# erthward/geonomics

Hardware: AMD Instinct MI355X
Metric: individual-timesteps/sec (higher is better)
Workload: dtype u64

## Files before the change

geonomics_amd/csrc/gnx_kernels_demog.hip:

```cpp
#include "gnx_internal.h"
#include <chrono>
#include "gnx_rng.h"
#include "gnx_compact.h"
#include "gnx_half.h"
#include "gnx_xo.h"

#define BIN_BLOCKS 512

__global__ void __launch_bounds__(256)
k_bins(int64_t n, const int32_t* n_dev, const float* x, const float* y, const uint8_t* ghost,
       double inv_hww, int nbx, int nby, int32_t* partials, GnxSetWords sw) {
  extern __shared__ int32_t lds_hist[];
  if (sw.dst && blockIdx.x == 0 && threadIdx.x < 4) sw.dst[threadIdx.x] = sw.v[threadIdx.x];
  if (n_dev) n = *n_dev;
  const int nb = nbx * nby;
  for (int k = threadIdx.x; k < nb; k += blockDim.x) lds_hist[k] = 0;
  __syncthreads();
  const int64_t stride = (int64_t)gridDim.x * blockDim.x;
  for (int64_t i = (int64_t)blockIdx.x * blockDim.x + threadIdx.x; i < n; i += stride) {
    if (ghost && ghost[i]) continue;
    int hx = min(nbx - 1, (int)floor((double)x[i] * inv_hww));
    int hy = min(nby - 1, (int)floor((double)y[i] * inv_hww));
    atomicAdd(&lds_hist[hy * nbx + hx], 1);
  }
// ... 645 lines not shown
                     n_max, (const int32_t*)h->cnt_dev, (const float*)h->mid_x,
                     (const float*)h->mid_y, (const uint8_t*)nullptr, 1.0 / L.hww, L.nbx, L.nby,
                     h->fb[2], GnxSetWords{});
  hipLaunchKernelGGL(k_lattice, dim3(1), dim3(256), lds_bytes, h->stream3, L.Jx, L.Jy, L.nbx,
                     (const int32_t*)h->fb[2], L.areas, L.hww, L.cprime, h->spl_P.c,
                     (int32_t*)nullptr, 0, (unsigned long long*)nullptr, 1, 1);
  HIPCHK(hipEventRecord(h->ev_latP, h->stream3));
  HIPCHK(hipGetLastError());
  h->latP_inflight = true;
  h->fb_zero[2] = true;
  h->spl_P.valid = true;
  return 0;
}

int gnx_l_bins_adults_async(gnx_state* h, const float* d_x, const float* d_y, int64_t N) {
  if (!(h->have_sp && gnx_fused_bins(h))) {
    h->fb_adults = false;
    return 0;
  }
  const GnxLattice& L = h->lat;
  const int nb = L.nbx * L.nby;
  const int cur = h->fb_cur;
  if (!h->fb_zero[cur])
    HIPCHK(hipMemsetAsync(h->fb[cur], 0, (size_t)nb * sizeof(int32_t), h->stream));
  h->fbp_x = d_x;
  h->fbp_y = d_y;
  h->fbp_N = N;
  h->fb_pending = true;
  h->fb_zero[cur] = false;
  h->fb_adults = true;
  h->fb_count = N;
  return 0;
}

int gnx_bins_adults_launch(gnx_state* h) {
  if (!h->fb_pending) return 0;
  h->fb_pending = false;
  const GnxLattice& L = h->lat;
  const int nb = L.nbx * L.nby;
  const int64_t N = h->fbp_N;
  const int blocks = (int)std::min<int64_t>(BIN_BLOCKS, std::max<int64_t>(1, (N + 255) / 256));
  hipLaunchKernelGGL(k_bins, dim3(blocks), dim3(256), (size_t)nb * sizeof(int32_t), h->stream3, N,
                     (const int32_t*)nullptr, h->fbp_x, h->fbp_y, (const uint8_t*)nullptr,
                     1.0 / L.hww, L.nbx, L.nby, h->fb[h->fb_cur], GnxSetWords{});
  HIPCHK(hipEventRecord(h->ev_binsN, h->stream3));
  HIPCHK(hipGetLastError());
  h->binsN_inflight = true;
  return 0;
}

void gnx_bins_adults_drop(gnx_state* h) {
  if (h->fb_pending) {
    h->fb_pending = false;
    h->fb_adults = false;
  }
}

int gnx_l_density_N(gnx_state* h) {
  GnxSoA s = h->soa[h->cur];
  if (!(gnx_fused_bins(h) && h->fb_adults && h->fb_count == h->N)) {
    h->fb_adults = false;
    h->nmax_ready = false;
    h->last_N_fused = false;
    return gnx_l_density(h, h->N, s.x, s.y, &h->spl_N, nullptr);
  }
  const GnxLattice& L = h->lat;
  const int64_t nn = (int64_t)L.Jx * L.Jy;
  const size_t lat_doubles = (size_t)4 * nn + std::max(L.Jx, L.Jy) + 1;
  const int nmax_R = gnx_nmax_rows_fit(L.Jx, lat_doubles);
  const size_t lds_bytes = (lat_doubles + gnx_nmax_lds_doubles(L.Jx, nmax_R)) * sizeof(double);
  const int cur = h->fb_cur;
  if (h->fb_pending) {
    HIPCHK(hipEventRecord(h->ev_perm, h->stream));
    HIPCHK(hipStreamWaitEvent(h->stream3, h->ev_perm, 0));
    GNXCHK(gnx_bins_adults_launch(h));
  }
  if (h->binsN_inflight) {
    HIPCHK(hipStreamWaitEvent(h->stream, h->ev_binsN, 0));
    h->binsN_inflight = false;
  }
  gnx_time_begin(h);
  hipLaunchKernelGGL(k_lattice_nmax, dim3(std::max(1, std::min(h->cfg.H, GNX_LATN_BLOCKS))), dim3(256),
                     lds_bytes, h->stream, L.Jx, L.Jy, L.nbx, (const int32_t*)h->fb[cur], L.areas,
                     L.hww, L.cprime, h->spl_N.c, h->cfg.W, h->cfg.H, h->nmax2 + cur,
                     h->fb[cur ^ 1], h->nmax2 + (cur ^ 1), (int32_t*)nullptr, (double*)nullptr,
                     GnxPubWords{}, nmax_R, gnx_nmax_scan_min());
  gnx_time_end(h, GNX_K_DENSITY, (double)h->N * 8.0);
  HIPCHK(hipGetLastError());
  h->spl_N.valid = true;
  h->nmax_cur = h->nmax2 + cur;
  h->nmax_ready = true;
  h->fb_zero[cur] = false;
  h->fb_zero[cur ^ 1] = true;
  h->fb_cur = cur ^ 1;
  h->fb_adults = false;
  h->last_N_fused = true;
  return 0;
}

bool gnx_l_lattices_tiled(gnx_state* h, bool have_pairs, const GnxPubWords& pub) {
  const GnxLattice& L = h->lat;
  const int64_t nn = (int64_t)L.Jx * L.Jy;
  const size_t lat_doubles = (size_t)4 * nn + std::max(L.Jx, L.Jy) + 1;
  const int nmax_R = gnx_nmax_rows_fit(L.Jx, lat_doubles);
  const size_t lds_bytes = (lat_doubles + gnx_nmax_lds_doubles(L.Jx, nmax_R)) * sizeof(double);
  if (lds_bytes > 64 * 1024 || !h->nmax_bits || !h->nmax_zeroed) return false;
  gnx_time_begin(h);
  hipLaunchKernelGGL(k_lattice_nmax,
                     dim3(std::max(1, std::min(h->cfg.H, GNX_LATN_BLOCKS)) + (have_pairs ? 1 : 0)),
                     dim3(256), lds_bytes, h->stream, L.Jx, L.Jy, L.nbx,
                     (const int32_t*)h->bin_partials, L.areas, L.hww, L.cprime, h->spl_N.c, h->cfg.W,
                     h->cfg.H, h->nmax_bits, (int32_t*)nullptr, (unsigned long long*)nullptr,
                     have_pairs ? h->bins_P : (int32_t*)nullptr, h->spl_P.c, pub, nmax_R, gnx_nmax_scan_min());
  gnx_time_end(h, GNX_K_DENSITY, (double)h->N * 8.0);
  h->spl_N.valid = true;
  h->spl_P.valid = have_pairs;
  h->nmax_cur = h->nmax_bits;
  h->nmax_ready = true;
  h->nmax_zeroed = false;
  return true;
}

int gnx_l_death_probs(gnx_state* h, bool with_selection) {
  int64_t N = h->N;
  if (N == 0) return 0;
  SplineC SN = make_splinec(h, h->spl_N), SP = make_splinec(h, h->spl_P);
  GNXCHK(gnx_wait_latP(h));
  gnx_time_begin(h);
  if (!h->nmax_ready) GNXCHK(launch_nmax(h));
  h->nmax_ready = false;
  hipLaunchKernelGGL(k_death_probs, dim3(gnx_grid(N, 256)), dim3(256), 0, h->stream,
                     make_deathp(h, with_selection), make_demp(h), SN, SP, h->soa[h->cur], h->rast,
                     gnx_trait_tab(h), h->delet_s, h->nmax_cur, h->p_death, h->d_cell);
  gnx_time_end(h, GNX_K_DEATH, (double)N * (28.0 + 8.0 * h->cfg.n_traits));
  HIPCHK(hipGetLastError());
  return 0;
}

__global__ void __launch_bounds__(256)
k_alive(int64_t N, const double* p_death, const uint8_t* dead_in, const int64_t* id,
        const uint8_t* ghost, const int32_t* grow, long long step, unsigned long long seed,
        int32_t* alive, int32_t* dead_row, int32_t* cnt, int stride, int64_t xo_first,
        int32_t* zero_jobs, const GnxDD* __restrict__ dd, GnxScanOut scan) {
  __shared__ int lds[16];
  __shared__ int lds2[8];
  const int64_t base = (int64_t)blockIdx.x * GNX_CB;
  if (dd) {
    N = (int64_t)dd->N + dd->B;
    step = dd->step;
    if (xo_first >= 0) xo_first = dd->N;
  }
  if (zero_jobs && blockIdx.x == 0 && threadIdx.x == 0) *zero_jobs = 0;
  bool fa[4], fd[4], fx[4];
#pragma unroll
  for (int r = 0; r < 4; ++r) {
    const int64_t i = base + r * 256 + threadIdx.x;
    fa[r] = fd[r] = fx[r] = false;
    if (i < N) {
      bool dead;
      const bool g = ghost[i] != 0;
      if (g) {
        dead = true;
      } else if (dead_in) {
        dead = dead_in[i] != 0;
      } else {
        uint4 rr = gnx_rand4(seed, (unsigned long long)id[i], step, OP_DEATH, 0);
        dead = (double)gnx_u01(rr.x) < p_death[i];
      }
      fa[r] = !dead;
      fd[r] = dead && !g && grow[i] >= 0;
      fx[r] = !dead && xo_first >= 0 && i >= xo_first && grow[i] < 0;
      alive[i] = (fa[r] ? 1 : 0) | (fx[r] ? 2 : 0);
      dead_row[i] = fd[r] ? 1 : 0;
    }
  }
  int rank[4], ta, td, tx;
  gnx_block_ranks(fa, rank, ta, lds);
  gnx_block_ranks(fd, rank, td, lds);
  gnx_block_ranks(fx, rank, tx, lds);
  if (scan.ticket) {
    const int v[3] = {ta, td, tx};
    gnx_count_and_scan<3>(v, cnt, scan, lds2);
    return;
  }
  if (threadIdx.x == 0) {
    cnt[blockIdx.x] = ta;
    cnt[stride + blockIdx.x] = td;
    cnt[2 * stride + blockIdx.x] = tx;
  }
}

struct GnxXoPlan {
  int32_t row;
  int32_t pop, job;
  int32_t prow[2];
  int32_t mixsel[2];
  int32_t ks[2];
  int32_t pad;
};

__global__ void __launch_bounds__(256)
k_xo_jobs_surv(int64_t N, int64_t first, int32_t* __restrict__ grow,
               const int32_t* __restrict__ alive, const int32_t* __restrict__ blk_off3,
               const int32_t* __restrict__ off_parent, const int32_t* __restrict__ off_keys,
               const uint8_t* __restrict__ off_start, const int32_t* __restrict__ free_rows,
               int64_t n_free, GnxHalves H, const int32_t* __restrict__ bp_off,
               const int32_t* __restrict__ bp_loci, int32_t* __restrict__ n_jobs,
               GnxXoPlan* __restrict__ plan) {
  __shared__ int lds[16];
  __shared__ int s_pop, s_job;
  const int64_t b = first / GNX_CB + blockIdx.x;
  const int64_t base = b * GNX_CB;
  bool fx[4];
#pragma unroll
  for (int r = 0; r < 4; ++r) {
    const int64_t i = base + r * 256 + threadIdx.x;
    fx[r] = i < N && (alive[i] & 2) != 0;
  }
  int rank[4], tot;
  gnx_block_ranks(fx, rank, tot, lds);
  const int32_t boff = blk_off3[b];
  const int NB = H.NB;
  const unsigned int all = (1u << NB) - 1u;
  int32_t row[4], prow[4][2], ks[4][2];
  int32_t par[4][2], key[4][2], st[4][2];
#pragma unroll
  for (int r = 0; r < 4; ++r) {
    const int64_t i = base + r * 256 + threadIdx.x;
    const int64_t k = fx[r] ? i - first : 0;
    row[r] = free_rows[n_free - 1 - (fx[r] ? boff + rank[r] : 0)];
#pragma unroll
    for (int p = 0; p < 2; ++p) {
      par[r][p] = off_parent[2 * k + p];
      key[r][p] = off_keys[2 * k + p];
      st[r][p] = off_start[2 * k + p];
    }
  }
  int32_t b0[4][2], b1[4][2];
#pragma unroll
  for (int r = 0; r < 4; ++r) {
    const int64_t i = base + r * 256 + threadIdx.x;
    if (fx[r]) grow[i] = row[r];
    else row[r] = -1;
#pragma unroll
    for (int p = 0; p < 2; ++p) {
      prow[r][p] = grow[par[r][p]];
      b0[r][p] = bp_off ? bp_off[key[r][p]] : 0;
      b1[r][p] = bp_off ? bp_off[key[r][p] + 1] : 0;
    }
  }
  unsigned int mixed[4][2], sel[4][2];
  int cf[4], cj[4];
#pragma unroll
  for (int r = 0; r < 4; ++r) {
    cf[r] = cj[r] = 0;
#pragma unroll
    for (int p = 0; p < 2; ++p) {
      if (!fx[r]) prow[r][p] = -1;
      ks[r][p] = key[r][p] * 2 + st[r][p];
      mixed[r][p] = all;
      sel[r][p] = 0u;
      if (fx[r] && prow[r][p] >= 0 && bp_off)
        gnx_block_masks(bp_loci + b0[r][p], b1[r][p] - b0[r][p], st[r][p], NB, H.BW, mixed[r][p],
                        sel[r][p]);
      if (fx[r]) {
        const int nf = __popc(mixed[r][p] & all);
        cf[r] += nf;
        cj[r] += prow[r][p] >= 0 ? nf : 0;
      }
    }
  }
  int of[4], oj[4], tf, tj;
  gnx_block_sums(cf, of, tf, lds);
  gnx_block_sums(cj, oj, tj, lds);
  if (threadIdx.x == 0) {
    s_pop = tf ? atomicSub(H.top, tf) : 0;
    s_job = tj ? atomicAdd(n_jobs, tj) : 0;
  }
  __syncthreads();
  const int pop0 = s_pop, job0 = s_job;
#pragma unroll
  for (int r = 0; r < 4; ++r) {
    const int64_t i = base + r * 256 + threadIdx.x;
    if (i < first || i >= N) continue;
    GnxXoPlan P;
    P.row = fx[r] ? row[r] : -1;
    P.pop = pop0 - 1 - of[r];
    P.job = job0 + oj[r];
#pragma unroll
    for (int p = 0; p < 2; ++p) {
      P.prow[p] = prow[r][p];
      P.mixsel[p] = (mixed[r][p] & 0xffffu) | (sel[r][p] << 16);
      P.ks[p] = ks[r][p];
    }
    plan[i - first] = P;
  }
}

__global__ void __launch_bounds__(256)
k_xo_jobs_write(int64_t B, GnxHalves H, const GnxXoPlan* __restrict__ plan,
                GnxXoJob* __restrict__ jobs) {
  const int NB = H.NB;
  const int64_t t = (int64_t)blockIdx.x * blockDim.x + threadIdx.x;
  if (t >= B * 2 * NB) return;
  const int64_t k = t / (2 * NB);
  const int rem = (int)(t - k * 2 * NB);
  const int p = rem / NB, q = rem - p * NB;
  const GnxXoPlan P = plan[k];
  if (P.row < 0) return;
  const unsigned int all = (1u << NB) - 1u;
  const unsigned int m0 = P.mixsel[0] & all, m1 = P.mixsel[1] & all;
  const unsigned int mixed = p ? m1 : m0, sel = (unsigned int)P.mixsel[p] >> 16;
  const unsigned int below = (1u << q) - 1u;
  const bool local = P.prow[p] >= 0;
  const int64_t lb = ((int64_t)P.row * 2 + p) * NB + q;
  const int64_t ph0 = (int64_t)(local ? P.prow[p] : 0) * 2 * NB;
  if ((mixed >> q) & 1u) {
    const int fr = (p ? __popc(m0) : 0) + __popc(mixed & below);
    const int jr = (p && P.prow[0] >= 0 ? __popc(m0) : 0) + __popc(mixed & below);
    const int32_t dst = H.stack[P.pop - fr];
    H.hmap[lb] = (int32_t)((uint32_t)dst | GNX_OWN);
    if (local) {
      GnxXoJob j;
      j.ph0 = GNX_BLK(H.hmap[ph0 + q]);
// ... 467 lines not shown
                       lds, lds2);
  }
}

__global__ void __launch_bounds__(256)
k_fill(int64_t cap, const int32_t* __restrict__ n_move, const int32_t* __restrict__ holes,
       const int32_t* __restrict__ movers, const int32_t* __restrict__ cnts, GnxSoA a, int n_layers,
       int n_traits, int tbw, const int32_t* __restrict__ rows_tmp, int32_t* __restrict__ free_rows,
       int64_t n_free, int has_rows, int xo, int32_t* __restrict__ newslot,
       const GnxDD* __restrict__ dd) {
  if (dd) n_free = dd->n_free;
  const int64_t stride = (int64_t)gridDim.x * blockDim.x;
  const int64_t t0 = (int64_t)blockIdx.x * blockDim.x + threadIdx.x;
  const int64_t H = *n_move;
  for (int64_t r = t0; r < H; r += stride) {
    const int64_t i = movers[r], k = holes[r];
    GnxRec rec = gnx_rec_load(a, i, cap, n_layers, n_traits, tbw);
    rec.ghost = 0;
    if (newslot) newslot[i] = (int32_t)k;
    gnx_rec_store(a, k, cap, n_layers, n_traits, tbw, rec);
    gnx_rec_rest(a, i, a, k, cap, n_layers, n_traits, tbw);
  }
  if (has_rows) {
    if (xo) n_free -= cnts[2];
    const int64_t D = cnts[1];
    for (int64_t r = t0; r < D; r += stride) free_rows[n_free + r] = rows_tmp[r];
  }
}

static bool jobs_fused_ok(const gnx_state* h) { return h->NB <= GNX_JF_NB; }

void gnx_launch_xo_jobs_surv(gnx_state* h, int64_t first_slot, const int32_t* d_alive,
                             const int32_t* d_blk_off, int buf) {
  const int64_t N = h->N;
  const int nbj = (int)((N - 1) / GNX_CB - first_slot / GNX_CB + 1);
  if (jobs_fused_ok(h)) {
    launch_jobs_fused(h, first_slot, d_alive, d_blk_off, buf);
    return;
  }
  h->jobs_inline[buf] = false;
  hipLaunchKernelGGL(k_xo_jobs_surv, dim3(nbj), dim3(256), 0, h->stream, N, first_slot,
                     h->soa[h->cur].grow, d_alive, d_blk_off + 2 * h->blk_stride, h->off_parent,
                     h->off_keys, h->off_start, h->free_rows, h->n_free, gnx_halves(h),
                     gnx_alias_bp(h), gnx_alias_loci(h), h->n_jobs_dev[buf], (GnxXoPlan*)h->xo_plan);
  const int64_t B = N - first_slot;
  hipLaunchKernelGGL(k_xo_jobs_write, dim3(gnx_grid(B * 2 * h->NB, 256)), dim3(256), 0, h->stream,
                     B, gnx_halves(h), (const GnxXoPlan*)h->xo_plan, (GnxXoJob*)h->jobs[buf]);
}

struct GnxDDEnd {
  GnxDD* dd;
  const int32_t* cnts;
  const int32_t* half_top;
  GnxDDRec* ring;
  int has_rows, xo;
  unsigned int* ticket;
};
__device__ __forceinline__ void gnx_dd_end_step(const GnxDDEnd& E) {
  GnxDD* dd = E.dd;
  const int32_t S = E.cnts[0], freed = E.cnts[1], X = E.xo ? E.cnts[2] : 0;
  GnxDDRec r;
  r.N0 = dd->N;
  r.P = dd->P;
  r.B = dd->B;
  r.S = S;
  r.xo = X;
  const int32_t n_free = dd->n_free - X + (E.has_rows ? freed : 0);
  r.n_free = n_free;
  r.half_top = E.half_top ? *E.half_top : 0;
  r.err = dd->err;
  r.max_id = dd->max_id + dd->B;
  r.step = dd->step;
  const int32_t seq = dd->seq + 1;
  dd->N = S;
  dd->ord_n = S;
  dd->n_free = n_free;
  dd->max_id = r.max_id;
  dd->step = dd->step + 1;
  dd->seq = seq;
  dd->P = 0;
  dd->B = 0;
  GnxDDRec* slot = E.ring + ((seq - 1) % GNX_DD_RING);
  __hip_atomic_store(&slot->seq, (int64_t)0, __ATOMIC_RELAXED, __HIP_MEMORY_SCOPE_SYSTEM);
  int64_t* w = (int64_t*)slot;
  const int64_t* v = (const int64_t*)&r;
  for (int k = 1; k < (int)(sizeof(GnxDDRec) / 8); ++k)
    __hip_atomic_store(&w[k], v[k], __ATOMIC_RELAXED, __HIP_MEMORY_SCOPE_SYSTEM);
  __hip_atomic_store(&slot->seq, (int64_t)seq, __ATOMIC_RELEASE, __HIP_MEMORY_SCOPE_SYSTEM);
}

__global__ void __launch_bounds__(256)
k_ord_flags(int64_t N, int64_t ord_n, const int32_t* __restrict__ ord,
            const int32_t* __restrict__ newslot, int32_t* __restrict__ cnt, GnxScanOut S,
            const GnxDD* __restrict__ dd, const int32_t* __restrict__ alive) {
  __shared__ int lds[16];
  __shared__ int lds2[8];
  if (dd) {
    N = (int64_t)dd->N + dd->B;
    ord_n = dd->ord_n;
  }
  gnx_ord_flags_body(N, ord_n, GnxOrdF{ord, alive ? nullptr : newslot, alive, cnt, S, ord_n, 0},
                     lds, lds2);
}

__global__ void __launch_bounds__(256)
k_ord_write(int64_t N, int64_t ord_n, const int32_t* __restrict__ ord,
            const int32_t* __restrict__ newslot, const int32_t* __restrict__ off,
            int32_t* __restrict__ ord_new, const GnxDD* __restrict__ dd, GnxDDEnd E,
            int tail_explicit, const int32_t* __restrict__ alive) {
  __shared__ int lds[16];
  __shared__ int last_s;
  if (dd) {
    N = (int64_t)dd->N + dd->B;
    ord_n = tail_explicit ? N : (int64_t)dd->ord_n;
  }
  const int64_t base = (int64_t)blockIdx.x * GNX_CB;
  bool f[4];
  int32_t ns[4];
#pragma unroll
  for (int r = 0; r < 4; ++r) {
    const int64_t k = base + r * 256 + threadIdx.x;
    if (alive) {
      const int32_t slot = k < N ? (int32_t)(k < ord_n ? ord[k] : k) : -1;
      ns[r] = (slot >= 0 && (alive[slot] & 1) != 0) ? slot : -1;
    } else {
      ns[r] = k < N ? newslot[k < ord_n ? ord[k] : k] : -1;
    }
    f[r] = ns[r] >= 0;
  }
  int rank[4], tot;
  gnx_block_ranks(f, rank, tot, lds);
  const int32_t o = off[blockIdx.x];
#pragma unroll
  for (int r = 0; r < 4; ++r)
    if (f[r]) ord_new[o + rank[r]] = ns[r];
  if (!E.dd) return;
  __syncthreads();
  if (threadIdx.x == 0) {
    const unsigned int t = __hip_atomic_fetch_add(E.ticket, 1u, __ATOMIC_RELAXED, __HIP_MEMORY_SCOPE_AGENT);
    last_s = t == gridDim.x - 1u;
    if (last_s) __hip_atomic_store(E.ticket, 0u, __ATOMIC_RELAXED, __HIP_MEMORY_SCOPE_AGENT);
  }
  __syncthreads();
  if (last_s && threadIdx.x == 0) gnx_dd_end_step(E);
}

__global__ void __launch_bounds__(256)
k_dead_rows(int64_t N, const int32_t* __restrict__ dead_row, const int32_t* __restrict__ blk_off_d,
            int32_t* __restrict__ grow, const int32_t* __restrict__ cnts, int xo,
            int32_t* __restrict__ free_rows, int64_t n_free) {
  __shared__ int lds[16];
  const int64_t base = (int64_t)blockIdx.x * GNX_CB;
  bool fd[4];
#pragma unroll
  for (int r = 0; r < 4; ++r) {
    const int64_t i = base + r * 256 + threadIdx.x;
    fd[r] = i < N && dead_row[i] != 0;
  }
  int rd[4], td;
  gnx_block_ranks(fd, rd, td, lds);
  if (xo) n_free -= cnts[2];
  const int32_t od = blk_off_d[blockIdx.x];
#pragma unroll
  for (int r = 0; r < 4; ++r) {
    const int64_t i = base + r * 256 + threadIdx.x;
    if (fd[r]) {
      free_rows[n_free + od + rd[r]] = grow[i];
      grow[i] = -1;
    }
  }
}

int gnx_l_mortality(gnx_state* h, const uint8_t* d_dead_inject, int64_t* deaths_out) {
  *deaths_out = 0;
  GNXCHK(gnx_l_mortality_enqueue(h, d_dead_inject));
  return gnx_l_mortality_finish(h, deaths_out);
}

int gnx_l_mortality_enqueue(gnx_state* h, const uint8_t* d_dead_inject) {
  int64_t N = h->N;
  h->mort_wait = false;
  gnx_bins_adults_drop(h);
  if (N == 0) return 0;
  const gnx_config& c = h->cfg;
  GnxSoA a = h->soa[h->cur], b = h->soa[h->cur ^ 1];
  const int nb = (int)((N + GNX_CB - 1) / GNX_CB);
  const bool xo = h->xo_deferred;
  const int64_t xo_first = h->xo_first, xo_B = xo ? h->xo_B : 0;
  const bool ord_keep = h->ord_mode && h->ord_valid && !h->tiled;
  int32_t* zero_jobs = nullptr;
  if (xo) {
    GNXCHK(gnx_xo_prepare_jobs(h, &zero_jobs));
    GNXCHK(gnx_half_reserve(h, 2 * (int64_t)h->NB * xo_B));
  }
  gnx_time_begin(h);
  hipLaunchKernelGGL(k_alive, dim3(nb), dim3(256), 0, h->stream, N, h->p_death, d_dead_inject,
                     a.id, a.ghost, a.grow, h->step, c.seed, h->flag, h->flag2, h->blk_cnt,
                     h->blk_stride, xo ? xo_first : (int64_t)-1, zero_jobs, (const GnxDD*)nullptr,
                     GnxScanOut{});
  const bool fill = h->compact_fill && h->stream3 != nullptr && d_dead_inject == nullptr;
  const bool side_scan = fill && xo && xo_B > 0 && jobs_fused_ok(h);
  const bool lazy_common = fill && h->sp.move && h->sp.mating_radius >= 0;
  const bool lazy_tile = lazy_common && gnx_env_int("GNX_TILE_LAZY", 0) != 0 && h->tile_lazy_ok &&
                         h->tile2_mode && h->tile_R * h->tile_C > 1 && !ord_keep;
  const bool lazy = lazy_tile || (lazy_common && h->eager_move && ord_keep && h->key_bits <= 24 &&
                                  h->n_ghost == 0 && !h->tile2_mode);
  const bool move_ahead = lazy && ord_keep && h->move_ahead_ok && h->stream2 != nullptr &&
                          h->xo_launch_late;
  const bool lazy_ord = lazy && ord_keep;
  if (side_scan || lazy_ord) HIPCHK(hipEventRecord(h->ev_alive, h->stream));
  if (side_scan) {
    HIPCHK(hipStreamWaitEvent(h->stream3, h->ev_alive, 0));
    GNXCHK(gnx_block_scan(h, 3, N, h->blk_cnt, h->blk_off, h->cnt_dev, h->h_pin_dev, 0, h->stream3));
    gnx_time_end(h, GNX_K_COMPACT, 0.0);
    HIPCHK(hipEventRecord(h->ev_counts, h->stream3));
  } else {
    GNXCHK(gnx_block_scan(h, 3, N, h->blk_cnt, h->blk_off, h->cnt_dev, h->h_pin_dev));
    gnx_time_end(h, GNX_K_COMPACT, 0.0);
    HIPCHK(hipEventRecord(h->ev_counts, h->stream));
  }
  h->jobs_self_scan = side_scan;
  int has_rows = (h->genomes_assigned && c.L > 0) ? 1 : 0;
  if (fill && !lazy) {
    if (!side_scan) HIPCHK(hipStreamWaitEvent(h->stream3, h->ev_counts, 0));
    hipLaunchKernelGGL(k_fill_lists, dim3(nb), dim3(256), 0, h->stream3, N, h->flag, h->flag2,
                       h->blk_off, h->blk_stride, h->cnt_dev, a.grow, has_rows,
                       (int32_t*)h->os_ktmp, (int32_t*)h->os_ktmp + c.cap_inds / 2,
                       (int32_t*)h->os_vtmp, ord_keep ? h->newslot : nullptr, h->fill_cnt,
                       (const GnxDD*)nullptr, GnxOrdF{});
    HIPCHK(hipEventRecord(h->ev_fill, h->stream3));
  }
  if (xo) {
    h->xo_deferred = false;
    GNXCHK(gnx_l_crossover_survivors(h, xo_first, xo_B, h->flag, h->blk_off));
    h->jobs_self_scan = false;
    if (h->xo_sort_waits && h->xo_wait_at == 2) GNXCHK(gnx_xo_wait_inflight(h));
  }
  if (move_ahead) GNXCHK(gnx_l_move_ahead(h, N));
  if (ord_keep && h->ord_inflight) HIPCHK(hipStreamWaitEvent(h->stream, h->ev_ord, 0));
  auto ord_launch = [&](hipStream_t os) {
    GnxScanOut So{h->ord_off, nullptr, nullptr, 0, nullptr, h->tickets + 2, h->blk_stride};
    hipLaunchKernelGGL(k_ord_flags, dim3(nb), dim3(256), 0, os, N, h->ord_n,
                       h->ord[h->ord_cur], h->newslot, h->ord_cnt, So, (const GnxDD*)nullptr,
                       lazy ? (const int32_t*)h->flag : (const int32_t*)nullptr);
    hipLaunchKernelGGL(k_ord_write, dim3(nb), dim3(256), 0, os, N, h->ord_n,
                       h->ord[h->ord_cur], h->newslot, h->ord_off, h->ord[h->ord_cur ^ 1],
                       (const GnxDD*)nullptr, GnxDDEnd{}, 0,
                       lazy ? (const int32_t*)h->flag : (const int32_t*)nullptr);
  };
  if (move_ahead) {
    ord_launch(h->stream);
    h->ord_inflight = false;
    h->ord_covers_xo = false;
    h->ord_cur ^= 1;
  }
  gnx_time_begin(h);
  const double rec_bytes = 34.0 + 4.0 * c.n_layers + 4.0 * c.n_traits + 16.0 * h->TW;
  if (lazy) {
    if (has_rows) {
      if (side_scan) HIPCHK(hipStreamWaitEvent(h->stream, h->ev_counts, 0));
      hipLaunchKernelGGL(k_dead_rows, dim3(nb), dim3(256), 0, h->stream, N,
                         (const int32_t*)h->flag2, (const int32_t*)(h->blk_off + h->blk_stride),
                         a.grow, (const int32_t*)h->cnt_dev, xo ? 1 : 0,
                         h->free_rows, h->n_free);
    }
    gnx_time_end(h, GNX_K_COMPACT, (double)N * 8.0);
    h->holes = true;
    h->holes_N = N;
    h->holes_flagged = N;
    ++h->pc[GNX_PC_LAZY_MORT];
  } else if (fill) {
    HIPCHK(hipStreamWaitEvent(h->stream, h->ev_fill, 0));
    const int64_t guess = std::max<int64_t>(h->fill_guess * 2, 4096);
    const int fb_ = (int)std::min<int64_t>(gnx_grid(std::min<int64_t>(guess, N), 256), 8192);
    hipLaunchKernelGGL(k_fill, dim3(fb_), dim3(256), 0, h->stream, c.cap_inds, h->fill_cnt,
                       (const int32_t*)h->os_ktmp, (const int32_t*)h->os_ktmp + c.cap_inds / 2,
                       h->cnt_dev, a, c.n_layers, c.n_traits, a.tb ? 2 * h->TW : 0,
                       (const int32_t*)h->os_vtmp, h->free_rows, h->n_free, has_rows, xo ? 1 : 0,
                       ord_keep ? h->newslot : nullptr, (const GnxDD*)nullptr);
    gnx_time_end(h, GNX_K_COMPACT, (double)N * 16.0 + (double)h->fill_guess * (16.0 + 2.0 * rec_bytes));
  } else {
    hipLaunchKernelGGL(k_compact, dim3(nb), dim3(256), 0, h->stream, N, c.cap_inds, h->flag,
                       h->flag2, h->blk_off, h->blk_stride, h->cnt_dev, a, b, c.n_layers, c.n_traits,
                       a.tb ? 2 * h->TW : 0, h->free_rows, h->n_free, has_rows, xo ? 1 : 0,
                       ord_keep ? h->newslot : nullptr);
    gnx_time_end(h, GNX_K_COMPACT, (double)N * (24.0 + 2.0 * rec_bytes));
  }
  if (move_ahead) {
  } else if (ord_keep) {
    if (!lazy_ord) {
      HIPCHK(hipEventRecord(h->ev_compact, h->stream));
      HIPCHK(hipStreamWaitEvent(h->stream3, h->ev_compact, 0));
    } else if (!side_scan) {
      HIPCHK(hipStreamWaitEvent(h->stream3, h->ev_alive, 0));
    }
    if (h->ord_inflight) h->ord_inflight = false;
    ord_launch(h->stream3);
    h->ord_covers_xo = false;
    if (h->xo_sort_waits && !h->xo_last_split && h->xo_ready_buf < 0) {
      for (int k = 0; k < 2; ++k)
        if (h->xo_inflight[k]) HIPCHK(hipStreamWaitEvent(h->stream3, h->ev_xo_done[k], 0));
      h->ord_covers_xo = true;
    }
    HIPCHK(hipEventRecord(h->ev_ord, h->stream3));
    h->ord_inflight = true;
    h->ord_cur ^= 1;
  } else {
    h->ord_valid = false;
  }
  HIPCHK(hipGetLastError());
  h->mort_wait = true;
  h->mort_xo = xo;
  h->mort_fill = fill;
  h->mort_ord_keep = ord_keep;
  h->mort_has_rows = has_rows;
  h->mort_N = N;
  return 0;
}

int gnx_l_mortality_finish(gnx_state* h, int64_t* deaths_out) {
// ... 191 lines not shown
```

geonomics_amd/csrc/gnx_kernels_pop.hip:

```cpp
#include "gnx_internal.h"
#include "gnx_rng.h"
#include "gnx_compact.h"
#include "gnx_tb.h"
#include "gnx_bins.h"

static int gnx_id_bits(const gnx_state* h) {
  int b = 1;
  while (b < 40 && (h->max_id >> b) != 0) ++b;
  return b;
}
static bool gnx_ord_sort(const gnx_state* h) {
  return h->ord_mode && h->ord_valid && !h->tiled;
}

__device__ __forceinline__ int wave_min_i(int v) {
#pragma unroll
  for (int m = 32; m >= 1; m >>= 1) v = min(v, __shfl_xor(v, m));
  return v;
}
__device__ __forceinline__ int wave_max_i(int v) {
#pragma unroll
  for (int m = 32; m >= 1; m >>= 1) v = max(v, __shfl_xor(v, m));
  return v;
}
// ... 1315 lines not shown
  if (n_dev) nb = (int)(((int64_t)*n_dev + GNX_CB - 1) / GNX_CB);
  if (dd) nb = (int)(((int64_t)dd->N + GNX_CB - 1) / GNX_CB);
  const int seg = (nb + 15) / 16;
  const int b0 = wave * seg, b1 = min(nb, b0 + seg);
  int run = 0;
  for (int b = b0; b < b1; ++b) run += blk_cnt[(int64_t)b * GNX_VTN + c];
  seg_tot[wave][c] = run;
  __syncthreads();
  int before = 0, total = 0;
  for (int w = 0; w < 16; ++w) {
    const int t = seg_tot[w][c];
    before += w < wave ? t : 0;
    total += t;
  }
  run = before;
  for (int b = b0; b < b1; ++b) {
    const int v = blk_cnt[(int64_t)b * GNX_VTN + c];
    blk_off[(int64_t)b * GNX_VTN + c] = run;
    run += v;
  }
  if (wave != 0) return;
  vt_count[c] = total;
  if (local) {
    int xs = total;
#pragma unroll
    for (int d = 1; d < 64; d <<= 1) {
      const int yv = __shfl_up(xs, d);
      if (c >= d) xs += yv;
    }
    vt_base[c] = (int64_t)(xs - total) * lam;
  }
}

struct GnxGoff {
  const int64_t* goff;
  const uint8_t* cls;
  const int32_t* rank;
  const int32_t* pblk;
  const int32_t* blk_off;
  const int64_t* vt_base;
  int64_t mul;
};

int gnx_vt_buffers(gnx_state* h) {
  if (h->vt_cls) return 0;
  const size_t cap = (size_t)h->cfg.cap_inds;
  const size_t nb = cap / GNX_CB + 2;
  HIPCHK(hipMalloc((void**)&h->vt_cls, cap));
  HIPCHK(hipMalloc((void**)&h->vt_scls, cap));
  HIPCHK(hipMalloc((void**)&h->vt_blk_nz, nb * sizeof(unsigned long long)));
  HIPCHK(hipMalloc((void**)&h->vt_rank, cap * sizeof(int32_t)));
  HIPCHK(hipMalloc((void**)&h->vt_pblk, cap * sizeof(int32_t)));
  HIPCHK(hipMalloc((void**)&h->vt_blk_cnt, nb * GNX_VTN * sizeof(int32_t)));
  HIPCHK(hipMalloc((void**)&h->vt_blk_off, nb * GNX_VTN * sizeof(int32_t)));
  HIPCHK(hipMalloc((void**)&h->vt_count, (GNX_VTN + GNX_MAX_TILES + 8) * sizeof(int32_t)));
  HIPCHK(hipMemset(h->vt_count, 0, (GNX_VTN + GNX_MAX_TILES + 8) * sizeof(int32_t)));
  HIPCHK(hipMalloc((void**)&h->vt_base, GNX_VTN * sizeof(int64_t)));
  return 0;
}

static GnxVtP gnx_vtp(const gnx_state* h) {
  const int vw = h->cfg.W / GNX_VT, vh = h->cfg.H / GNX_VT;
  return GnxVtP{vw, vh, 1.0f / (float)vw, 1.0f / (float)vh};
}

static int gnx_vt_out(gnx_state* h, GnxVtOut* out) {
  *out = GnxVtOut{nullptr, nullptr, nullptr, 0, nullptr, nullptr, nullptr, nullptr, 0, 1,
                  GnxVtP{1, 1, 1.f, 1.f}};
  h->vt_fused = false;
  if (h->id_order != 1 || !h->sp.n_births_fixed || h->sp.mating_radius < 0) return 0;
  GNXCHK(gnx_vt_buffers(h));
  *out = GnxVtOut{h->vt_scls, h->vt_blk_cnt, h->vt_blk_nz, (int)(h->cfg.cap_inds / GNX_CB + 2),
                  h->vt_count, h->vt_cls, h->vt_rank, h->vt_base,
                  h->tiled ? 0 : 1, (int64_t)h->sp.n_births_lambda, gnx_vtp(h)};
  h->vt_fused = true;
  return 0;
}

int gnx_l_pair_cls(gnx_state* h, int64_t P, bool local) {
  GNXCHK(gnx_vt_buffers(h));
  GnxSoA s = h->soa[h->cur];
  if (h->sp.n_births_fixed) {
    if (!h->vt_fused && h->N > 0 && P != 0) {
      gnx_set_error("tile-major offspring ids: the pair list was made without its classification");
      return 1;
    }
    if (local != !h->tiled) {
      gnx_set_error("tile-major offspring ids: the bases' owner does not match the tile grid");
      return 1;
    }
    h->vt_mul = (int64_t)h->sp.n_births_lambda;
    h->vt_weighted = false;
    if (h->N == 0 || P == 0)
      HIPCHK(hipMemsetAsync(h->vt_count, 0, GNX_VTN * sizeof(int32_t), h->stream));
    h->pair_goff_local_base = local;
    h->pair_goff_ready = true;
    return 0;
  }
  int nb;
  {
    h->vt_weighted = true;
    nb = (int)((P + GNX_CB - 1) / GNX_CB);
    h->vt_mul = 1;
    if (P > 0)
      hipLaunchKernelGGL(k_pair_cls, dim3(nb), dim3(256), 0, h->stream, P, (const int32_t*)nullptr,
                         (const int32_t*)h->pairs, (const float*)s.x, (const float*)s.y,
                         (const int32_t*)h->nbirths, gnx_vtp(h), h->vt_cls, h->vt_rank, h->vt_pblk,
                         h->vt_blk_cnt);
  }
  if (P == 0) nb = 0;
  hipLaunchKernelGGL(k_cls_scan, dim3(1), dim3(1024), 0, h->stream, nb, (const int32_t*)nullptr,
                     (const GnxDD*)nullptr, (const int32_t*)h->vt_blk_cnt, h->vt_blk_off,
                     h->vt_count, h->vt_base, local ? 1 : 0, h->vt_mul);
  HIPCHK(hipGetLastError());
  h->pair_goff_local_base = local;
  h->pair_goff_ready = true;
  return 0;
}

static GnxGoff gnx_goff_vt(const gnx_state* h) {
  if (!h->vt_weighted)
    return GnxGoff{nullptr, h->vt_cls, h->vt_rank, nullptr, nullptr, h->vt_base, h->vt_mul};
  return GnxGoff{nullptr, h->vt_cls, h->vt_rank, h->vt_pblk, h->vt_blk_off, h->vt_base, h->vt_mul};
}

struct PairP {
  int64_t N;
  const int32_t* focal;
  const int32_t* mate;
  const uint8_t* keep_in;
  float b;
  int sexed, ra_f, ra_m, dedup;
  long long step;
  unsigned long long seed;
  const GnxDD* dd;
};

__device__ __forceinline__ bool pair_ok(const PairP& P, const GnxSoA& s, int64_t i) {
  const int m = P.mate[i];
  if (m < 0) return false;
  const int fo = P.focal ? P.focal[i] : (int)i;
  bool keep;
  if (P.keep_in) {
    keep = P.keep_in[i] != 0;
  } else {
    uint4 r = gnx_rand4(P.seed, (unsigned long long)s.id[i], P.step, OP_PAIR_KEEP, 0);
    keep = gnx_u01(r.x) < P.b;
  }
  bool ok = keep;
  if (P.sexed) ok = ok && (s.sex[fo] == 0) && (s.sex[m] == 1);
  return ok && (s.age[fo] >= P.ra_f) && (s.age[m] >= P.ra_m);
}

__global__ void __launch_bounds__(256)
k_pair_flags(PairP P, GnxSoA s, int32_t* flag2, int32_t* cnt, GnxVtOut vt) {
  __shared__ int lds[16];
  __shared__ int vtot[GNX_VTN];
  if (vt.scls && threadIdx.x < GNX_VTN) vtot[threadIdx.x] = 0;
  const int64_t base = (int64_t)blockIdx.x * GNX_CB;
  P.N = gnx_dd_n(P.dd, P.N);
  P.step = gnx_dd_step(P.dd, P.step);
  bool f[4];
  float px[4] = {0.f, 0.f, 0.f, 0.f}, py[4] = {0.f, 0.f, 0.f, 0.f};
  if (vt.scls) {
#pragma unroll
    for (int r = 0; r < 4; ++r) {
      const int64_t i = base + r * 256 + threadIdx.x;
      if (i < P.N) {
        px[r] = s.x[i];
        py[r] = s.y[i];
      }
    }
  }
#pragma unroll
  for (int r = 0; r < 4; ++r) {
    const int64_t i = base + r * 256 + threadIdx.x;
    f[r] = false;
    if (i < P.N) {
      bool ok = pair_ok(P, s, i);
      if (ok && P.dedup) {
        const int m = P.mate[i];
        if (P.mate[m] == (int32_t)i && s.id[m] < s.id[i] && pair_ok(P, s, m)) ok = false;
      }
      if (s.ghost[P.focal ? P.focal[i] : (int)i]) ok = false;
      f[r] = ok;
      flag2[i] = ok ? 1 : 0;
    }
  }
  int rank[4], tot;
  gnx_block_ranks(f, rank, tot, lds);
  if (threadIdx.x == 0) cnt[blockIdx.x] = tot;
  if (!vt.scls) return;
  const int lane = threadIdx.x & 63;
#pragma unroll
  for (int r = 0; r < 4; ++r) {
    const int64_t i = base + r * 256 + threadIdx.x;
    int c = GNX_VTN;
    if (f[r]) {
      c = gnx_vt_of(vt.V, px[r], py[r]);
      vt.scls[i] = (uint8_t)c;
    }
    unsigned long long todo = __ballot(f[r]);
    while (todo) {
      const int leader = __ffsll((long long)todo) - 1;
      const int lc = __shfl(c, leader);
      const unsigned long long same = __ballot(f[r] && c == lc);
      if (lane == leader) atomicAdd(&vtot[lc], __popcll(same));
      todo &= ~same;
    }
  }
  __syncthreads();
  if (threadIdx.x < GNX_VTN) {
    const int t = vtot[threadIdx.x];
    vt.blk_cnt[(int64_t)threadIdx.x * vt.stride + blockIdx.x] = t;
    if (t) atomicAdd(&vt.total[threadIdx.x], t);
    const unsigned long long nz = __ballot(t != 0);
    if (threadIdx.x == 0) vt.blk_nz[blockIdx.x] = nz;
  }
}

__global__ void __launch_bounds__(256)
k_pair_compact(int64_t N, const int32_t* focal, const int32_t* mate, const int32_t* flag2,
               const int32_t* blk_off, const float* x, const float* y, const uint64_t* popkey,
               int idbits, int32_t* pairs, float* mid_x, float* mid_y, uint64_t* key,
               const int32_t* __restrict__ cnt, int32_t* __restrict__ total_dev,
               int64_t* __restrict__ host, long long seq, const int32_t* __restrict__ extra,
               GnxDD* __restrict__ dd, int dd_births, int64_t dd_cap, GnxBinP bins, GnxVtOut vt) {
  __shared__ int lds[16];
  __shared__ int psum[4];
  __shared__ int vcnt[16][GNX_VTN];
  __shared__ int vpre[GNX_VTN];
  if (dd) N = dd->N;
  if (vt.cls) {
    for (int k = threadIdx.x; k < 16 * GNX_VTN; k += 256) (&vcnt[0][0])[k] = 0;
    const int lane = threadIdx.x & 63, wave = threadIdx.x >> 6;
    unsigned long long nz = vt.blk_nz[blockIdx.x];
    for (int k = 0; nz; ++k) {
      const int c = __ffsll((long long)nz) - 1;
      nz &= nz - 1;
      if ((k & 3) != wave) continue;
      const int32_t* row = vt.blk_cnt + (int64_t)c * vt.stride;
      int part = 0;
      for (int b2 = lane; b2 < (int)blockIdx.x; b2 += 64) part += row[b2];
#pragma unroll
      for (int d = 32; d > 0; d >>= 1) part += __shfl_xor(part, d);
      if (lane == 0) vpre[c] = part;
    }
    if (vt.local && blockIdx.x == 0 && wave == 3) {
      const int tot = vt.total[lane];
      int xs = tot;
#pragma unroll
      for (int d = 1; d < 64; d <<= 1) {
        const int yv = __shfl_up(xs, d);
        if (lane >= d) xs += yv;
      }
      vt.base[lane] = (int64_t)(xs - tot) * vt.lam;
    }
  }
  int self_off = 0;
  if (cnt) {
    const int lane = threadIdx.x & 63, wave = threadIdx.x >> 6;
    const int upto = blockIdx.x == 0 ? (int)gridDim.x : (int)blockIdx.x;
    int part = 0;
    for (int i = threadIdx.x; i < upto; i += 256) part += cnt[i];
#pragma unroll
    for (int d = 32; d > 0; d >>= 1) part += __shfl_xor(part, d);
    if (lane == 0) psum[wave] = part;
    __syncthreads();
    const int sum = psum[0] + psum[1] + psum[2] + psum[3];
    self_off = blockIdx.x == 0 ? 0 : sum;
    if (blockIdx.x == 0 && threadIdx.x == 0) {
      *total_dev = sum;
      if (dd) {
        int64_t births = (int64_t)sum * dd_births;
        if ((int64_t)dd->N + births > dd_cap) {
          dd->err |= GNX_DD_ERR_SLOTS;
          births = 0;
        }
        dd->P = sum;
        dd->B = (int32_t)births;
      }
      if (host) {
        __hip_atomic_store(&host[0], (int64_t)sum, __ATOMIC_RELAXED, __HIP_MEMORY_SCOPE_SYSTEM);
        if (extra)
          __hip_atomic_store(&host[12], (int64_t)*extra, __ATOMIC_RELAXED, __HIP_MEMORY_SCOPE_SYSTEM);
        asm volatile("s_waitcnt vmcnt(0)" ::: "memory");
        if (seq)
          __hip_atomic_store(&host[3], (int64_t)seq, __ATOMIC_RELAXED, __HIP_MEMORY_SCOPE_SYSTEM);
      }
    }
  }
  const int64_t base = (int64_t)blockIdx.x * GNX_CB;
  bool f[4];
  int sc[4] = {0, 0, 0, 0};
#pragma unroll
  for (int r = 0; r < 4; ++r) {
    const int64_t i = base + r * 256 + threadIdx.x;
    f[r] = i < N && flag2[i] != 0;
    if (vt.cls && i < N) sc[r] = vt.scls[i];
  }
  int rank[4], tot;
  gnx_block_ranks(f, rank, tot, lds);
  int vc[4] = {0, 0, 0, 0}, vrw[4] = {0, 0, 0, 0};
  float fx[4], fy[4];
  int fo4[4];
#pragma unroll
  for (int r = 0; r < 4; ++r) {
    const int64_t i = base + r * 256 + threadIdx.x;
    fo4[r] = f[r] ? (focal ? focal[i] : (int)i) : 0;
    fx[r] = f[r] ? x[fo4[r]] : 0.f;
    fy[r] = f[r] ? y[fo4[r]] : 0.f;
  }
  if (vt.cls) {
    const int lane = threadIdx.x & 63, wave = threadIdx.x >> 6;
#pragma unroll
    for (int r = 0; r < 4; ++r) {
      vc[r] = f[r] ? sc[r] : GNX_VTN;
      gnx_vt_wave_ranks<false>(f[r], vc[r], 1, lane, vcnt[r * 4 + wave], vrw[r]);
    }
    __syncthreads();
  }
  const int32_t bo = cnt ? self_off : blk_off[blockIdx.x];
#pragma unroll
  for (int r = 0; r < 4; ++r) {
    const int64_t i = base + r * 256 + threadIdx.x;
    int bin = 0;
    if (f[r]) {
      const int p = bo + rank[r];
      const int m = mate[i];
      const int fo = fo4[r];
      pairs[2 * p] = fo;
      pairs[2 * p + 1] = m;
      const float mx = (fx[r] + x[m]) / 2.0f, my = (fy[r] + y[m]) / 2.0f;
      mid_x[p] = mx;
      mid_y[p] = my;
      const uint64_t k = popkey[i];
      key[p] = ((k >> idbits) << 40) | (k & ((1ull << idbits) - 1ull));
      if (bins.bins) bin = gnx_bin_of(bins, mx, my);
      if (vt.cls) {
        const int wave = threadIdx.x >> 6;
// ... 624 lines not shown
```

Baseline: 2.529 billion.

## Batch global loads ahead of compute in alive, dead-row and pair-flag kernels

The alive, dead-row and pair-flag kernels now issue all per-element global loads for their four rows up front into registers, clamping indices to stay in bounds, and only then compute. This lets many loads be in flight at once instead of each row's compute waiting on its own dependent loads. k_pair_flags is restructured to gather mate, focal, age, sex and ghost values in staged batches, and it checks the reciprocal-mate dedup only when some lane needs it. That kernel also gets a waves-per-EU occupancy hint, which trades register pressure against occupancy and could force spills given the larger register arrays.

```diff
diff --git a/geonomics_amd/csrc/gnx_kernels_demog.hip b/geonomics_amd/csrc/gnx_kernels_demog.hip
--- a/geonomics_amd/csrc/gnx_kernels_demog.hip
+++ b/geonomics_amd/csrc/gnx_kernels_demog.hip
@@ -821,24 +821,42 @@
   }
   if (zero_jobs && blockIdx.x == 0 && threadIdx.x == 0) *zero_jobs = 0;
   bool fa[4], fd[4], fx[4];
+  uint8_t gh[4] = {0, 0, 0, 0}, din[4] = {0, 0, 0, 0};
+  int64_t idv[4] = {0, 0, 0, 0};
+  double pd[4] = {0.0, 0.0, 0.0, 0.0};
+  int32_t gr[4] = {0, 0, 0, 0};
+  if (base < N) {
+#pragma unroll
+    for (int r = 0; r < 4; ++r) {
+      const int64_t ic = min(base + r * 256 + (int64_t)threadIdx.x, N - 1);
+      gh[r] = ghost[ic];
+      gr[r] = grow[ic];
+      if (dead_in) {
+        din[r] = dead_in[ic];
+      } else {
+        idv[r] = id[ic];
+        pd[r] = p_death[ic];
+      }
+    }
+  }
 #pragma unroll
   for (int r = 0; r < 4; ++r) {
     const int64_t i = base + r * 256 + threadIdx.x;
     fa[r] = fd[r] = fx[r] = false;
     if (i < N) {
       bool dead;
-      const bool g = ghost[i] != 0;
+      const bool g = gh[r] != 0;
       if (g) {
         dead = true;
       } else if (dead_in) {
-        dead = dead_in[i] != 0;
+        dead = din[r] != 0;
       } else {
-        uint4 rr = gnx_rand4(seed, (unsigned long long)id[i], step, OP_DEATH, 0);
-        dead = (double)gnx_u01(rr.x) < p_death[i];
+        uint4 rr = gnx_rand4(seed, (unsigned long long)idv[r], step, OP_DEATH, 0);
+        dead = (double)gnx_u01(rr.x) < pd[r];
       }
       fa[r] = !dead;
-      fd[r] = dead && !g && grow[i] >= 0;
-      fx[r] = !dead && xo_first >= 0 && i >= xo_first && grow[i] < 0;
+      fd[r] = dead && !g && gr[r] >= 0;
+      fx[r] = !dead && xo_first >= 0 && i >= xo_first && gr[r] < 0;
       alive[i] = (fa[r] ? 1 : 0) | (fx[r] ? 2 : 0);
       dead_row[i] = fd[r] ? 1 : 0;
     }
@@ -1612,20 +1630,30 @@
   __shared__ int lds[16];
   const int64_t base = (int64_t)blockIdx.x * GNX_CB;
   bool fd[4];
+  const int32_t popped = xo ? cnts[2] : 0;
+  const int32_t od = blk_off_d[blockIdx.x];
+  int32_t dr[4] = {0, 0, 0, 0}, gr[4] = {-1, -1, -1, -1};
+  if (base < N) {
+#pragma unroll
+    for (int r = 0; r < 4; ++r) {
+      const int64_t ic = min(base + r * 256 + (int64_t)threadIdx.x, N - 1);
+      dr[r] = dead_row[ic];
+      gr[r] = grow[ic];
+    }
+  }
 #pragma unroll
   for (int r = 0; r < 4; ++r) {
     const int64_t i = base + r * 256 + threadIdx.x;
-    fd[r] = i < N && dead_row[i] != 0;
+    fd[r] = i < N && dr[r] != 0;
   }
   int rd[4], td;
   gnx_block_ranks(fd, rd, td, lds);
-  if (xo) n_free -= cnts[2];
-  const int32_t od = blk_off_d[blockIdx.x];
+  n_free -= popped;
 #pragma unroll
   for (int r = 0; r < 4; ++r) {
     const int64_t i = base + r * 256 + threadIdx.x;
     if (fd[r]) {
-      free_rows[n_free + od + rd[r]] = grow[i];
+      free_rows[n_free + od + rd[r]] = gr[r];
       grow[i] = -1;
     }
   }
diff --git a/geonomics_amd/csrc/gnx_kernels_pop.hip b/geonomics_amd/csrc/gnx_kernels_pop.hip
--- a/geonomics_amd/csrc/gnx_kernels_pop.hip
+++ b/geonomics_amd/csrc/gnx_kernels_pop.hip
@@ -1491,7 +1491,7 @@
   return ok && (s.age[fo] >= P.ra_f) && (s.age[m] >= P.ra_m);
 }
 
-__global__ void __launch_bounds__(256)
+__global__ void __launch_bounds__(256) __attribute__((amdgpu_waves_per_eu(8, 8)))
 k_pair_flags(PairP P, GnxSoA s, int32_t* flag2, int32_t* cnt, GnxVtOut vt) {
   __shared__ int lds[16];
   __shared__ int vtot[GNX_VTN];
@@ -1501,30 +1501,84 @@
   P.step = gnx_dd_step(P.dd, P.step);
   bool f[4];
   float px[4] = {0.f, 0.f, 0.f, 0.f}, py[4] = {0.f, 0.f, 0.f, 0.f};
-  if (vt.scls) {
+  if (vt.scls && base < P.N) {
+#pragma unroll
+    for (int r = 0; r < 4; ++r) {
+      const int64_t ic = min(base + r * 256 + (int64_t)threadIdx.x, P.N - 1);
+      px[r] = s.x[ic];
+      py[r] = s.y[ic];
+    }
+  }
+  const bool draw = P.focal != nullptr && P.keep_in == nullptr;
+  int32_t mt[4] = {-1, -1, -1, -1}, fo4[4] = {0, 0, 0, 0};
+  int64_t idi[4] = {0, 0, 0, 0};
+  uint8_t kin[4] = {1, 1, 1, 1};
+  int32_t age_f[4] = {0, 0, 0, 0}, age_m[4] = {0, 0, 0, 0}, mm[4] = {-1, -1, -1, -1};
+  uint8_t sex_f[4] = {0, 0, 0, 0}, sex_m[4] = {0, 0, 0, 0}, gh[4] = {0, 0, 0, 0};
+  bool ok4[4] = {false, false, false, false};
+  if (base < P.N) {
+#pragma unroll
+    for (int r = 0; r < 4; ++r) {
+      const int64_t ic = min(base + r * 256 + (int64_t)threadIdx.x, P.N - 1);
+      mt[r] = P.mate[ic];
+      fo4[r] = P.focal ? P.focal[ic] : (int32_t)ic;
+      if (draw || P.dedup) idi[r] = s.id[ic];
+      if (P.focal && P.keep_in) kin[r] = P.keep_in[ic];
+    }
+#pragma unroll
+    for (int r = 0; r < 4; ++r) {
+      age_f[r] = s.age[fo4[r]];
+      gh[r] = s.ghost[fo4[r]];
+      if (P.sexed) sex_f[r] = s.sex[fo4[r]];
+    }
+#pragma unroll
+    for (int r = 0; r < 4; ++r) {
+      const int32_t mc = mt[r] >= 0 ? mt[r] : fo4[r];
+      age_m[r] = s.age[mc];
+      if (P.sexed) sex_m[r] = s.sex[mc];
+      if (P.dedup) mm[r] = P.mate[mc];
+    }
+  }
+  bool recip = false;
+#pragma unroll
+  for (int r = 0; r < 4; ++r) {
+    const int64_t i = base + r * 256 + threadIdx.x;
+    bool ok = i < P.N && mt[r] >= 0;
+    if (P.focal) {
+      bool keep = kin[r] != 0;
+      if (draw) {
+        uint4 rr = gnx_rand4(P.seed, (unsigned long long)idi[r], P.step, OP_PAIR_KEEP, 0);
+        keep = gnx_u01(rr.x) < P.b;
+      }
+      ok = ok && keep;
+    }
+    if (P.sexed) ok = ok && sex_f[r] == 0 && sex_m[r] == 1;
+    ok4[r] = ok && age_f[r] >= P.ra_f && age_m[r] >= P.ra_m;
+    recip = recip || (ok4[r] && P.dedup && mm[r] == (int32_t)i);
+  }
+  if (recip) {
+    int64_t idm[4];
+#pragma unroll
+    for (int r = 0; r < 4; ++r) idm[r] = s.id[mt[r] >= 0 ? mt[r] : fo4[r]];
 #pragma unroll
     for (int r = 0; r < 4; ++r) {
       const int64_t i = base + r * 256 + threadIdx.x;
-      if (i < P.N) {
-        px[r] = s.x[i];
-        py[r] = s.y[i];
-      }
+      if (!(ok4[r] && mm[r] == (int32_t)i && idm[r] < idi[r])) continue;
+      bool okm;
+      if (P.focal) {
+        okm = pair_ok(P, s, mt[r]);
+      } else {
+        okm = age_m[r] >= P.ra_f && age_f[r] >= P.ra_m;
+        if (P.sexed) okm = okm && sex_m[r] == 0 && sex_f[r] == 1;
+      }
+      if (okm) ok4[r] = false;
     }
   }
 #pragma unroll
   for (int r = 0; r < 4; ++r) {
     const int64_t i = base + r * 256 + threadIdx.x;
-    f[r] = false;
-    if (i < P.N) {
-      bool ok = pair_ok(P, s, i);
-      if (ok && P.dedup) {
-        const int m = P.mate[i];
-        if (P.mate[m] == (int32_t)i && s.id[m] < s.id[i] && pair_ok(P, s, m)) ok = false;
-      }
-      if (s.ghost[P.focal ? P.focal[i] : (int)i]) ok = false;
-      f[r] = ok;
-      flag2[i] = ok ? 1 : 0;
-    }
+    f[r] = ok4[r] && gh[r] == 0;
+    if (i < P.N) flag2[i] = f[r] ? 1 : 0;
   }
   int rank[4], tot;
   gnx_block_ranks(f, rank, tot, lds);
```

Result: faster. 2.590 billion, median of 6 (+2.4%).
